# Stansfash/nonstationary-precip

Measured on AMD Instinct MI355X. Metric: dsvi_elbo_steps_per_sec, higher is better.
Workload: dtype f32; 1 GPU; 2-layer DSVI DeepGP (hidden 3->2 + last 2->1), M=1024, S=10, minibatch 4096 (global, split over the GPUs) of synthetic N=1e5 spatio-temporal grid; fwd+ELBO+bwd+Adam; M=1024, S=10, per_gpu_batch=4096, global_batch=4096, N=100000, parallelism=dp1, kzz_cholesky_dtype=f64, hipgraph=True

## Files before the change

nonstationary-precip_amd/csrc/gemm_i8.hip:

```cpp
#include <cstdlib>
#include "common.h"

namespace {

#ifndef NSGP_I8_DMA
#define NSGP_I8_DMA 1
#endif
constexpr int I8_BM = 128, I8_BN = 64, I8_BK = 32;
constexpr int I8_SW = 5;

typedef int v4i __attribute__((ext_vector_type(4)));
typedef int v16i __attribute__((ext_vector_type(16)));

__global__ __launch_bounds__(256) void i8_slice_w_kernel(const double* __restrict__ W, int64_t M, int64_t Mp, int64_t KB,
                                                         signed char* __restrict__ Wd, double* __restrict__ wsc) {
    __shared__ double lds[4];
    const int64_t b = blockIdx.y, m = blockIdx.x;
    signed char* out = Wd + b * (int64_t)I8_SW * KB * 2 * Mp * 16;
    const int64_t plane = KB * 2 * Mp * 16;
    if (m >= M) {
        for (int64_t k = threadIdx.x; k < KB * 32; k += 256)
            for (int a = 0; a < I8_SW; ++a) out[a * plane + ((k >> 5) * 2 + ((k >> 4) & 1)) * Mp * 16 + m * 16 + (k & 15)] = 0;
        return;
    }
    const double* row = W + (b * M + m) * M;
    const auto nmax = [](double a, double c) { return (a > c || a != a) ? a : c; };
    double mx = 0.0;
    for (int64_t k = threadIdx.x; k <= m; k += 256) mx = nmax(fabs(row[k]), mx);
    for (int off = 32; off > 0; off >>= 1) mx = nmax(__shfl_xor(mx, off, 64), mx);
    if ((threadIdx.x & 63) == 0) lds[threadIdx.x >> 6] = mx;
    __syncthreads();
    mx = nmax(nmax(lds[0], lds[1]), nmax(lds[2], lds[3]));
    const bool fin = mx <= 1.7976931348623157e308;
    int e = 0;
    (void)frexp(fin ? mx : 0.0, &e);
    const double rs = (fin && mx > 0.0) ? ldexp(1.0, e) : 1.0;
    if (threadIdx.x == 0) wsc[b * M + m] = fin ? rs / 64.0 : __builtin_nan("");
    const double inv = 64.0 / rs;
    for (int64_t k = threadIdx.x; k < KB * 32; k += 256) {
        double t = (fin && k <= m && k < M) ? row[k] * inv : 0.0;
        const int64_t o = ((k >> 5) * 2 + ((k >> 4) & 1)) * Mp * 16 + m * 16 + (k & 15);
#pragma unroll
        for (int a = 0; a < I8_SW; ++a) {
            const double d = rint(t);
            out[a * plane + o] = (signed char)(int)d;
            t = (t - d) * 128.0;
        }
    }
}

template <int D, int SK>
__global__ __launch_bounds__(256) void i8_rbf_build_kernel(const float* __restrict__ Z, const float* __restrict__ x, int64_t sx,
                                                           const float* __restrict__ ls, const float* __restrict__ os,
                                                           int64_t M, int64_t n, int64_t np, int64_t KB,
                                                           signed char* __restrict__ Kd, double* __restrict__ ksc,
                                                           float* __restrict__ Kf) {
    const int64_t b = blockIdx.z, kb = blockIdx.y;
    const int64_t j = (int64_t)blockIdx.x * 256 + threadIdx.x;
    __shared__ double zs[32][D];
    __shared__ int bad;
    if (threadIdx.x == 0) bad = 0;
    if (threadIdx.x < 32 * D) {
        const int kk = threadIdx.x / D, d = threadIdx.x % D;
        const int64_t k = kb * 32 + kk;
        zs[kk][d] = k < M ? (double)Z[(b * M + k) * D + d] / (double)ls[b * D + d] : 0.0;
    }
    __syncthreads();
    const double osd = (double)os[b];
    bool fin = fabs(osd) <= 1.7976931348623157e308;
#pragma unroll
    for (int d = 0; d < D; ++d) fin = fin && fabs((double)ls[b * D + d]) <= 1.7976931348623157e308;
    int e = 0;
    (void)frexp(fin ? osd : 0.0, &e);
    const double cs = ldexp(1.0, e);
    const double sc = fin ? osd * 64.0 / cs : 0.0;
    if (j < np) {
        double xs[D];
#pragma unroll
        for (int d = 0; d < D; ++d) xs[d] = j < n ? (double)x[b * sx + j * D + d] / (double)ls[b * D + d] : 0.0;
        signed char* out = Kd + b * (int64_t)SK * KB * 2 * np * 16;
        const int64_t plane = KB * 2 * np * 16;
#pragma unroll
        for (int h = 0; h < 2; ++h) {
            int pk[SK][4] = {};
#pragma unroll
            for (int q = 0; q < 16; ++q) {
                const int kk = h * 16 + q;
                double r2 = 0.0;
#pragma unroll
                for (int d = 0; d < D; ++d) { const double df = zs[kk][d] - xs[d]; r2 = __builtin_fma(df, df, r2); }
                const bool in = j < n && kb * 32 + kk < M;
                const bool nan_e = in && r2 != r2;
                if (nan_e) bad = 1;
                const double ev = in ? t_fexp<double>(-0.5 * r2) : 0.0;
                const double evd = nan_e ? 0.0 : ev;
                if (Kf && in) Kf[(b * M + kb * 32 + kk) * n + j] = (float)(osd * ev);
                double t = sc * evd;
#pragma unroll
                for (int s = 0; s < SK; ++s) {
                    const double dg = rint(t);
                    pk[s][q >> 2] |= ((int)dg & 0xFF) << (8 * (q & 3));
                    t = (t - dg) * 128.0;
                }
            }
#pragma unroll
            for (int s = 0; s < SK; ++s) {
                v4i v = {pk[s][0], pk[s][1], pk[s][2], pk[s][3]};
                *reinterpret_cast<v4i*>(out + s * plane + (kb * 2 + h) * np * 16 + j * 16) = v;
            }
        }
    }
    __syncthreads();
    if (threadIdx.x == 0)
        ksc[(b * KB + kb) * gridDim.x + blockIdx.x] = (fin && !bad) ? cs / 64.0 : __builtin_nan("");
}

template <int P64, int SK, int LEV>
__global__ __launch_bounds__(256, 2) void i8_proj_kernel(const signed char* __restrict__ Wd, const double* __restrict__ wsc,
                                                         const signed char* __restrict__ Kd, const double* __restrict__ ksc,
                                                         const float* __restrict__ rv, int64_t M, int64_t n, int64_t Mp,
                                                         int64_t np, int64_t KB, int tiles_n, float* __restrict__ Y,
                                                         void* __restrict__ p0, void* __restrict__ p1, int part_rows) {
    extern __shared__ __attribute__((aligned(16))) unsigned char i8_smem[];
    constexpr int A_STAGE = I8_SW * 2 * I8_BM * 16, B_STAGE = SK * 2 * I8_BN * 16;
    unsigned char* As = i8_smem;
    unsigned char* Bs = i8_smem + 2 * A_STAGE;
    double* Ws = reinterpret_cast<double*>(i8_smem + 2 * (A_STAGE + B_STAGE));
    float* Rs = reinterpret_cast<float*>(Ws + I8_BM);
    const int tid = threadIdx.x, lane = tid & 63, wave = __builtin_amdgcn_readfirstlane(tid >> 6);
    const int wm0 = (wave >> 1) * 64, wn0 = (wave & 1) * 32;
    const int64_t bb = blockIdx.y;
    const int tiles_m = (int)(Mp / I8_BM);
    const int bm = tiles_m - 1 - (int)blockIdx.x / tiles_n;
    const int bn = (int)blockIdx.x % tiles_n;
    const int64_t m0 = (int64_t)bm * I8_BM, n0 = (int64_t)bn * I8_BN;
    int nkb = (int)((m0 + I8_BM) / I8_BK);
    if (nkb > KB) nkb = (int)KB;
    const signed char* Wb = Wd + bb * (int64_t)I8_SW * KB * 2 * Mp * 16;
    const signed char* Kb = Kd + bb * (int64_t)SK * KB * 2 * np * 16;
    const int64_t wplane = KB * 2 * Mp * 16, kplane = KB * 2 * np * 16;

    const signed char* ga[5];
#pragma unroll
    for (int j = 0; j < 5; ++j) {
        const int q = tid + 256 * j;
        const int a = q >> 8, h = (q >> 7) & 1, row = q & 127;
        ga[j] = Wb + a * wplane + (int64_t)h * Mp * 16 + (m0 + row) * 16;
    }
    constexpr int NPB = (SK * 128 + 255) / 256;
    const signed char* gb[NPB];
#pragma unroll
    for (int j = 0; j < NPB; ++j) {
        int q = tid + 256 * j;
        if (q >= SK * 128) q = SK * 128 - 1;
        const int s = q >> 7, h = (q >> 6) & 1, col = q & 63;
        gb[j] = Kb + s * kplane + (int64_t)h * np * 16 + (n0 + col) * 16;
    }
    const int64_t astep = 2 * Mp * 16, bstep = 2 * np * 16;
#if NSGP_I8_DMA
    typedef const __attribute__((address_space(1))) void* gptr_t;
    typedef __attribute__((address_space(3))) void* lptr_t;
    auto dma = [&](int kb, int buf) __attribute__((always_inline)) {
#pragma unroll
        for (int j = 0; j < 5; ++j)
            __builtin_amdgcn_global_load_lds((gptr_t)(ga[j] + (int64_t)kb * astep),
                                             (lptr_t)(As + buf * A_STAGE + (wave * 64 + 256 * j) * 16), 16, 0, 0);
#pragma unroll
        for (int j = 0; j < NPB; ++j)
            if (wave * 64 + 256 * j < SK * 128)
                __builtin_amdgcn_global_load_lds((gptr_t)(gb[j] + (int64_t)kb * bstep),
                                                 (lptr_t)(Bs + buf * B_STAGE + (wave * 64 + 256 * j) * 16), 16, 0, 0);
    };
#endif
    v4i ra[5], rb[NPB];
    auto gload = [&](int kb) __attribute__((always_inline)) {
#pragma unroll
        for (int j = 0; j < 5; ++j) ra[j] = *reinterpret_cast<const v4i*>(ga[j] + (int64_t)kb * astep);
#pragma unroll
        for (int j = 0; j < NPB; ++j) rb[j] = *reinterpret_cast<const v4i*>(gb[j] + (int64_t)kb * bstep);
    };
    auto sstore = [&](int buf) __attribute__((always_inline)) {
#pragma unroll
        for (int j = 0; j < 5; ++j) *reinterpret_cast<v4i*>(As + buf * A_STAGE + (tid + 256 * j) * 16) = ra[j];
#pragma unroll
        for (int j = 0; j < NPB; ++j)
            if (tid + 256 * j < SK * 128) *reinterpret_cast<v4i*>(Bs + buf * B_STAGE + (tid + 256 * j) * 16) = rb[j];
    };

    v16i acc[LEV][2];
#pragma unroll
    for (int l = 0; l < LEV; ++l)
#pragma unroll
        for (int i = 0; i < 2; ++i)
#pragma unroll
            for (int r = 0; r < 16; ++r) acc[l][i][r] = 0;

    const int wave_nkb = __builtin_amdgcn_readfirstlane((int)((m0 + wm0 + 64 + I8_BK - 1) / I8_BK));
    const int half = lane >> 5, lr = lane & 31;
    const int64_t gx = (np + 255) >> 8;
    const double* ks = ksc + bb * KB * gx + (n0 >> 8);
    const float* rvb = rv ? rv + bb * M : nullptr;
#if NSGP_I8_DMA
    dma(0, 0);
#else
    gload(0);
    sstore(0);
#endif
    const double kslot = ks[(int64_t)(tid < nkb ? tid : nkb - 1) * gx];
    const int64_t prow = m0 + (tid & (I8_BM - 1)), crow = prow < M ? prow : M - 1;
    const double wload = wsc[bb * M + crow];
    const float rload = rvb ? rvb[crow] : 0.0f;
    const double wrow = prow < M ? wload : 0.0;
    const float rrow = prow < M ? rload : 0.0f;
    if (tid < I8_BM) { Ws[tid] = wrow; Rs[tid] = rrow; }
#if NSGP_I8_DMA
    asm volatile("s_waitcnt vmcnt(0)" ::: "memory");
#endif
    const double kscale = __syncthreads_or(kslot != kslot) ? __builtin_nan("") : ks[0];
    for (int kb = 0; kb < nkb; ++kb) {
        const int buf = kb & 1;
#if NSGP_I8_DMA
        if (kb + 1 < nkb) dma(kb + 1, buf ^ 1);
#else
        if (kb + 1 < nkb) gload(kb + 1);
#endif
        if (kb < wave_nkb) {
            v4i af[2][2], bf[SK];
#pragma unroll
            for (int s = 0; s < SK; ++s)
                bf[s] = *reinterpret_cast<const v4i*>(Bs + buf * B_STAGE + ((s * 2 + half) * I8_BN + wn0 + lr) * 16);
#pragma unroll
            for (int i = 0; i < 2; ++i)
                af[0][i] = *reinterpret_cast<const v4i*>(As + buf * A_STAGE + ((0 * 2 + half) * I8_BM + wm0 + 32 * i + lr) * 16);
#pragma unroll
            for (int a = 0; a < I8_SW; ++a) {
                if (a + 1 < I8_SW) {
#pragma unroll
                    for (int i = 0; i < 2; ++i)
                        af[(a + 1) & 1][i] = *reinterpret_cast<const v4i*>(
                            As + buf * A_STAGE + (((a + 1) * 2 + half) * I8_BM + wm0 + 32 * i + lr) * 16);
                }
#pragma unroll
                for (int s = 0; s < SK; ++s)
                    if (a + s < LEV) {
#pragma unroll
                        for (int i = 0; i < 2; ++i)
                            acc[a + s][i] = __builtin_amdgcn_mfma_i32_32x32x32_i8(af[a & 1][i], bf[s], acc[a + s][i], 0, 0, 0);
                    }
            }
        }
#if NSGP_I8_DMA
        asm volatile("s_waitcnt vmcnt(0)" ::: "memory");
#else
        if (kb + 1 < nkb) sstore(buf ^ 1);
#endif
        __syncthreads();
    }

    double sdot = 0.0, ssq = 0.0;
    const int64_t col = n0 + wn0 + lr;
#pragma unroll
    for (int i = 0; i < 2; ++i)
#pragma unroll
        for (int r = 0; r < 16; ++r) {
            const int lrow = wm0 + 32 * i + (r & 3) + 8 * (r >> 2) + 4 * half;
            const int64_t row = m0 + lrow;
            const double wr = Ws[lrow];
            const float rr = Rs[lrow];
            double v = (double)acc[LEV - 1][i][r];
#pragma unroll
            for (int l = LEV - 2; l >= 0; --l) v = __builtin_fma(v, 0.0078125, (double)acc[l][i][r]);
            const bool in = row < M && col < n;
            v *= (in ? wr : 0.0) * kscale;
            if (in) Y[(bb * M + row) * n + col] = (float)v;
            sdot += v * ((rvb && in) ? (double)rr : 0.0);
            ssq += v * v;
        }
    sdot += __shfl_xor(sdot, 32, 64);
    ssq += __shfl_xor(ssq, 32, 64);
    double* red = reinterpret_cast<double*>(i8_smem);
    __syncthreads();
    if (lane < 32) {
        red[(0 + (wave >> 1)) * I8_BN + wn0 + lane] = sdot;
        red[(2 + (wave >> 1)) * I8_BN + wn0 + lane] = ssq;
    }
    __syncthreads();
    if (tid < I8_BN && n0 + tid < n) {
        const int64_t o = (bb * part_rows + bm) * n + n0 + tid;
        const double d = red[tid] + red[I8_BN + tid], q = red[2 * I8_BN + tid] + red[3 * I8_BN + tid];
        if (P64) {
            if (p0) reinterpret_cast<double*>(p0)[o] = d;
            reinterpret_cast<double*>(p1)[o] = q;
        } else {
            if (p0) reinterpret_cast<float*>(p0)[o] = (float)d;
            reinterpret_cast<float*>(p1)[o] = (float)q;
        }
    }
}

static inline int64_t i8_mp(int64_t M) { return cdiv64(M, I8_BM) * I8_BM; }
static inline int64_t i8_np(int64_t n) { return cdiv64(n, I8_BN) * I8_BN; }
static inline int64_t i8_kb(int64_t M) { return cdiv64(M, I8_BK); }

}

extern "C" {

int nsgp_i8_supported(int64_t M) { return (M >= 1 && M <= 4096) ? 1 : 0; }
size_t nsgp_i8_w_planes_bytes(int64_t batch, int64_t M) {
    return (batch > 0 && M > 0) ? (size_t)(batch * I8_SW * i8_kb(M) * 2 * i8_mp(M) * 16) : 0;
}
size_t nsgp_i8_k_planes_bytes(int64_t batch, int64_t M, int64_t n, int planes) {
    return (batch > 0 && M > 0 && n > 0 && (planes == 4 || planes == 5)) ? (size_t)(batch * planes * i8_kb(M) * 2 * i8_np(n) * 16) : 0;
}
size_t nsgp_i8_tiles(int64_t M) { return M > 0 ? (size_t)cdiv64(M, I8_BM) : 0; }
size_t nsgp_i8_kscale_count(int64_t batch, int64_t M, int64_t n) {
    return (batch > 0 && M > 0 && n > 0) ? (size_t)(batch * i8_kb(M) * cdiv64(i8_np(n), 256)) : 0;
}

int nsgp_i8_slice_w_f64(const double* W, int64_t batch, int64_t M, void* Wd, double* wscale, void* stream) {
    if (!W) return -1; if (batch < 0) return -2; if (M < 0 || !nsgp_i8_supported(M > 0 ? M : 1)) return -3;
    if (!Wd) return -4; if (!wscale) return -5;
    if (batch == 0 || M == 0) return 0;
    if (batch > 65535) return -2;
    hipLaunchKernelGGL(i8_slice_w_kernel, dim3((unsigned)i8_mp(M), (unsigned)batch), dim3(256), 0, (hipStream_t)stream, W, M,
                       i8_mp(M), i8_kb(M), (signed char*)Wd, wscale);
    return nsgp_launch_status();
}

int nsgp_i8_rbf_build_f32(const float* Z, const float* x, int64_t x_batch_stride, const float* ls, const float* os,
                          int64_t batch, int64_t M, int64_t n, int D, int planes, void* Kd, double* kscale, float* Kzx_f32,
                          void* stream) {
    if (planes != 4 && planes != 5) return -10;
    if (!Z) return -1; if (!x) return -2; if (x_batch_stride < 0) return -3; if (!ls) return -4; if (!os) return -5;
    if (batch < 0) return -6; if (M < 0 || !nsgp_i8_supported(M > 0 ? M : 1)) return -7; if (n < 0) return -8;
    if (D < 1 || D > 4) return -9; if (!Kd) return -10; if (!kscale) return -11;
    if (batch == 0 || M == 0 || n == 0) return 0;
    if (batch > 65535 || i8_kb(M) > 65535) return -6;
    const int64_t np = i8_np(n), KB = i8_kb(M);
    dim3 grid((unsigned)cdiv64(np, 256), (unsigned)KB, (unsigned)batch);
    hipStream_t st = (hipStream_t)stream;
    signed char* kd = (signed char*)Kd;
#define NSGP_I8_BUILD(DD, SS) hipLaunchKernelGGL((i8_rbf_build_kernel<DD, SS>), grid, dim3(256), 0, st, Z, x, x_batch_stride, ls, os, M, n, np, KB, kd, kscale, Kzx_f32)
    if (planes == 4) {
        switch (D) { case 1: NSGP_I8_BUILD(1, 4); break; case 2: NSGP_I8_BUILD(2, 4); break; case 3: NSGP_I8_BUILD(3, 4); break;
                     default: NSGP_I8_BUILD(4, 4); break; }
    } else {
        switch (D) { case 1: NSGP_I8_BUILD(1, 5); break; case 2: NSGP_I8_BUILD(2, 5); break; case 3: NSGP_I8_BUILD(3, 5); break;
                     default: NSGP_I8_BUILD(4, 5); break; }
    }
#undef NSGP_I8_BUILD
    return nsgp_launch_status();
}

int nsgp_svgp_tri_gemm_colstats_i8(const void* Wd, const double* wscale, const void* Kd, const double* kscale,
                                   int planes, const float* rowvec, int64_t batch, int64_t M, int64_t n, float* Y,
                                   void* part_dot, void* part_sq, int64_t part_rows, int partials_f64, void* stream) {
    if (planes != 4 && planes != 5) return -5;
    if (!Wd) return -1; if (!wscale) return -2; if (!Kd) return -3; if (!kscale) return -4;
    if (batch < 0) return -6; if (M < 0 || !nsgp_i8_supported(M > 0 ? M : 1)) return -7; if (n < 0) return -8;
    if (!Y) return -9; if (!part_sq) return -11; if (part_rows < cdiv64(M > 0 ? M : 1, I8_BM)) return -12;
    if (batch == 0 || M == 0 || n == 0) return 0;
    const int64_t Mp = i8_mp(M), np = i8_np(n), KB = i8_kb(M);
    const int64_t tiles_n = np / I8_BN, tiles = (Mp / I8_BM) * tiles_n;
    if (tiles > 2147483647LL || batch > 65535) return -8;
    const size_t lds = 2 * (size_t)(I8_SW * 2 * I8_BM * 16 + planes * 2 * I8_BN * 16) + I8_BM * (sizeof(double) + sizeof(float));
    hipStream_t st = (hipStream_t)stream;
    dim3 grid((unsigned)tiles, (unsigned)batch);
#define NSGP_I8_PROJ(PP, SS) hipLaunchKernelGGL((i8_proj_kernel<PP, SS, (SS == 5 ? 6 : 5)>), grid, dim3(256), lds, st, (const signed char*)Wd, wscale, \
        (const signed char*)Kd, kscale, rowvec, M, n, Mp, np, KB, (int)tiles_n, Y, part_dot, part_sq, (int)part_rows)
    if (planes == 4) { if (partials_f64) NSGP_I8_PROJ(1, 4); else NSGP_I8_PROJ(0, 4); }
    else { if (partials_f64) NSGP_I8_PROJ(1, 5); else NSGP_I8_PROJ(0, 5); }
#undef NSGP_I8_PROJ
    return nsgp_launch_status();
}

}
```

Before: 239.9 steps/s.

## Make int8 projection GEMM persistent with 128x128 tiles and multi-stage DMA pipeline

Reworks the int8 sliced triangular projection kernel into a persistent kernel. It launches one 512-thread workgroup per CU, and each workgroup walks tiles in a serpentine order. The N tile grows from 64 to 128 columns and the inner loop gets a configurable stage pipeline using direct global-to-LDS loads with vmcnt-based waits. The next tile's prologue loads overlap the current tile's epilogue. The aim is to cut launch/tail imbalance and global-load stalls and to raise reuse of the A planes. In exchange it uses more LDS per block, lowers occupancy, and adds hand-written waitcnt and barrier logic.

```diff
diff --git a/nonstationary-precip_amd/csrc/gemm_i8.hip b/nonstationary-precip_amd/csrc/gemm_i8.hip
--- a/nonstationary-precip_amd/csrc/gemm_i8.hip
+++ b/nonstationary-precip_amd/csrc/gemm_i8.hip
@@ -3,10 +3,12 @@
 
 namespace {
 
-#ifndef NSGP_I8_DMA
-#define NSGP_I8_DMA 1
+#ifndef NSGP_I8_STAGES
+#define NSGP_I8_STAGES 2
 #endif
-constexpr int I8_BM = 128, I8_BN = 64, I8_BK = 32;
+constexpr int I8_BM = 128, I8_BN = 128, I8_BK = 32;
+constexpr int I8_NPAD = 64;
+constexpr int I8_STAGES = NSGP_I8_STAGES;
 constexpr int I8_SW = 5;
 
 typedef int v4i __attribute__((ext_vector_type(4)));
@@ -115,192 +117,245 @@
         ksc[(b * KB + kb) * gridDim.x + blockIdx.x] = (fin && !bad) ? cs / 64.0 : __builtin_nan("");
 }
 
+template <int N> __device__ __forceinline__ void i8_vmwait() { asm volatile("s_waitcnt vmcnt(%0)" ::"n"(N) : "memory"); }
+__device__ __forceinline__ void i8_barrier() { asm volatile("s_waitcnt lgkmcnt(0)\n\ts_barrier" ::: "memory"); }
+
 template <int P64, int SK, int LEV>
-__global__ __launch_bounds__(256, 2) void i8_proj_kernel(const signed char* __restrict__ Wd, const double* __restrict__ wsc,
-                                                         const signed char* __restrict__ Kd, const double* __restrict__ ksc,
-                                                         const float* __restrict__ rv, int64_t M, int64_t n, int64_t Mp,
-                                                         int64_t np, int64_t KB, int tiles_n, float* __restrict__ Y,
-                                                         void* __restrict__ p0, void* __restrict__ p1, int part_rows) {
+__global__ __launch_bounds__(512) void i8_proj_kernel(const signed char* __restrict__ Wd, const double* __restrict__ wsc,
+                                                      const signed char* __restrict__ Kd, const double* __restrict__ ksc,
+                                                      const float* __restrict__ rv, int64_t M, int64_t n, int64_t Mp,
+                                                      int64_t np, int64_t KB, int tiles_n, int tiles_row, int total,
+                                                      float* __restrict__ Y, void* __restrict__ p0, void* __restrict__ p1,
+                                                      int part_rows) {
     extern __shared__ __attribute__((aligned(16))) unsigned char i8_smem[];
-    constexpr int A_STAGE = I8_SW * 2 * I8_BM * 16, B_STAGE = SK * 2 * I8_BN * 16;
-    unsigned char* As = i8_smem;
-    unsigned char* Bs = i8_smem + 2 * A_STAGE;
-    double* Ws = reinterpret_cast<double*>(i8_smem + 2 * (A_STAGE + B_STAGE));
+    constexpr int NST = I8_STAGES, DEPTH = NST - 1;
+    constexpr int A_STAGE = I8_SW * 2 * I8_BM * 16, STAGE = A_STAGE + SK * 2 * I8_BN * 16;
+    constexpr int ACH = A_STAGE / 1024, NCH = STAGE / 1024, NJ = (NCH + 7) / 8;
+    static_assert(DEPTH >= 1 && DEPTH <= 3 && 8 * (NJ - 1) < NCH, "chunk schedule");
+    double* red = reinterpret_cast<double*>(i8_smem + NST * STAGE);
+    double* Ws = red + 4 * I8_BN;
     float* Rs = reinterpret_cast<float*>(Ws + I8_BM);
+    int* Fl = reinterpret_cast<int*>(Rs + I8_BM);
     const int tid = threadIdx.x, lane = tid & 63, wave = __builtin_amdgcn_readfirstlane(tid >> 6);
-    const int wm0 = (wave >> 1) * 64, wn0 = (wave & 1) * 32;
-    const int64_t bb = blockIdx.y;
-    const int tiles_m = (int)(Mp / I8_BM);
-    const int bm = tiles_m - 1 - (int)blockIdx.x / tiles_n;
-    const int bn = (int)blockIdx.x % tiles_n;
-    const int64_t m0 = (int64_t)bm * I8_BM, n0 = (int64_t)bn * I8_BN;
-    int nkb = (int)((m0 + I8_BM) / I8_BK);
-    if (nkb > KB) nkb = (int)KB;
-    const signed char* Wb = Wd + bb * (int64_t)I8_SW * KB * 2 * Mp * 16;
-    const signed char* Kb = Kd + bb * (int64_t)SK * KB * 2 * np * 16;
+    const int wm0 = (wave >> 2) * 64, wn0 = (wave & 3) * 32;
+    const int halfl = lane >> 5, lrl = lane & 31;
     const int64_t wplane = KB * 2 * Mp * 16, kplane = KB * 2 * np * 16;
-
-    const signed char* ga[5];
-#pragma unroll
-    for (int j = 0; j < 5; ++j) {
-        const int q = tid + 256 * j;
-        const int a = q >> 8, h = (q >> 7) & 1, row = q & 127;
-        ga[j] = Wb + a * wplane + (int64_t)h * Mp * 16 + (m0 + row) * 16;
-    }
-    constexpr int NPB = (SK * 128 + 255) / 256;
-    const signed char* gb[NPB];
-#pragma unroll
-    for (int j = 0; j < NPB; ++j) {
-        int q = tid + 256 * j;
-        if (q >= SK * 128) q = SK * 128 - 1;
-        const int s = q >> 7, h = (q >> 6) & 1, col = q & 63;
-        gb[j] = Kb + s * kplane + (int64_t)h * np * 16 + (n0 + col) * 16;
-    }
     const int64_t astep = 2 * Mp * 16, bstep = 2 * np * 16;
-#if NSGP_I8_DMA
+    const int64_t gx = (np + 255) >> 8;
+    const bool last_dma = NCH % 8 == 0 || wave + 8 * (NJ - 1) < NCH;
+
+    int bm = 0, nkb = 0, wave_nkb = 0;
+    int64_t bb = 0, m0 = 0, n0 = 0;
+    const signed char* g[NJ];
+    int64_t gstep[NJ];
+    unsigned voffa = 0, voffb = 0;
+    double kslot = 0.0, ks0 = 0.0, wload = 0.0;
+    float rload = 0.0f;
+
     typedef const __attribute__((address_space(1))) void* gptr_t;
     typedef __attribute__((address_space(3))) void* lptr_t;
-    auto dma = [&](int kb, int buf) __attribute__((always_inline)) {
-#pragma unroll
-        for (int j = 0; j < 5; ++j)
-            __builtin_amdgcn_global_load_lds((gptr_t)(ga[j] + (int64_t)kb * astep),
-                                             (lptr_t)(As + buf * A_STAGE + (wave * 64 + 256 * j) * 16), 16, 0, 0);
-#pragma unroll
-        for (int j = 0; j < NPB; ++j)
-            if (wave * 64 + 256 * j < SK * 128)
-                __builtin_amdgcn_global_load_lds((gptr_t)(gb[j] + (int64_t)kb * bstep),
-                                                 (lptr_t)(Bs + buf * B_STAGE + (wave * 64 + 256 * j) * 16), 16, 0, 0);
+    auto dma = [&](int kb, int st) __attribute__((always_inline)) {
+#pragma unroll
+        for (int j = 0; j < NJ; ++j)
+            if (j < NJ - 1 || last_dma) {
+                const signed char* base = g[j] + (int64_t)kb * gstep[j];
+                unsigned voff = wave + 8 * j < ACH ? voffa : voffb;
+                asm volatile("" : "+s"(base), "+v"(voff));
+                __builtin_amdgcn_global_load_lds((gptr_t)(base + voff),
+                                                 (lptr_t)(i8_smem + st * STAGE + (wave + 8 * j) * 1024), 16, 0, 0);
+            }
     };
+    auto wait_stages = [&](int k) __attribute__((always_inline)) {
+        if (k <= 0) i8_vmwait<0>();
+        else if (k == 1) { if (last_dma) i8_vmwait<NJ>(); else i8_vmwait<NJ - 1>(); }
+        else if (k == 2) { if (last_dma) i8_vmwait<2 * NJ>(); else i8_vmwait<2 * (NJ - 1)>(); }
+        else { if (last_dma) i8_vmwait<3 * NJ>(); else i8_vmwait<3 * (NJ - 1)>(); }
+    };
+    auto begin_tile = [&](int t) __attribute__((always_inline)) {
+        const int q = (int)((unsigned)t / (unsigned)tiles_row), r = t - q * tiles_row;
+        bm = (int)(Mp / I8_BM) - 1 - q;
+        bb = (int)((unsigned)r / (unsigned)tiles_n);
+        const int bn = r - (int)bb * tiles_n;
+        m0 = (int64_t)bm * I8_BM, n0 = (int64_t)bn * I8_BN;
+        nkb = (int)((m0 + I8_BM) / I8_BK);
+        if (nkb > KB) nkb = (int)KB;
+        wave_nkb = __builtin_amdgcn_readfirstlane((int)((m0 + wm0 + 64 + I8_BK - 1) / I8_BK));
+        const signed char* Wb = Wd + bb * (int64_t)I8_SW * KB * 2 * Mp * 16;
+        const signed char* Kb = Kd + bb * (int64_t)SK * KB * 2 * np * 16;
+#pragma unroll
+        for (int j = 0; j < NJ; ++j) {
+            int c = wave + 8 * j;
+            if (c >= NCH) c = NCH - 1;
+            if (c < ACH) {
+                g[j] = Wb + (c >> 2) * wplane + (int64_t)((c >> 1) & 1) * Mp * 16 + (m0 + (c & 1) * 64) * 16;
+                gstep[j] = astep;
+            } else {
+                const int cb = c - ACH;
+                g[j] = Kb + (cb >> 2) * kplane + (int64_t)((cb >> 1) & 1) * np * 16;
+                gstep[j] = bstep;
+            }
+        }
+        voffa = (unsigned)lane * 16u;
+        {
+            int64_t col = n0 + (wave & 1) * 64 + lane;
+            if (col >= np) col = np - 1;
+            voffb = (unsigned)col * 16u;
+        }
+#pragma unroll
+        for (int d = 0; d < DEPTH; ++d)
+            if (d < nkb) dma(d, d);
+        const double* ks = ksc + bb * KB * gx + (n0 >> 8);
+        kslot = ks[(int64_t)(tid < nkb ? tid : nkb - 1) * gx];
+        ks0 = ks[0];
+        const int64_t prow = m0 + (tid & (I8_BM - 1)), crow = prow < M ? prow : M - 1;
+        wload = wsc[bb * M + crow];
+        rload = rv ? rv[bb * M + crow] : 0.0f;
+    };
+
+    const int G = (int)gridDim.x, wg = (int)blockIdx.x;
+    const auto tile_of = [&](int j) { return (int64_t)j * G + ((j & 1) ? G - 1 - wg : wg); };
+    int round = 0;
+    begin_tile((int)tile_of(0));
+    for (;;) {
+        {
+            int tid = (int)threadIdx.x;
+            asm volatile("" : "+v"(tid));
+            const int64_t prow = m0 + (tid & (I8_BM - 1));
+            const double wrow = prow < M ? wload : 0.0;
+            const float rrow = prow < M ? rload : 0.0f;
+            if (tid < I8_BM) { Ws[tid] = wrow; Rs[tid] = rrow; }
+            const bool anynan = __builtin_amdgcn_ballot_w64(kslot != kslot) != 0;
+            if (wave < 2 && lane == 0) Fl[wave] = anynan ? 1 : 0;
+        }
+        i8_vmwait<0>();
+        i8_barrier();
+        const double kscale = (Fl[0] | Fl[1]) ? __builtin_nan("") : ks0;
+
+        v16i acc[LEV][2];
+#pragma unroll
+        for (int l = 0; l < LEV; ++l)
+#pragma unroll
+            for (int i = 0; i < 2; ++i)
+#pragma unroll
+                for (int r = 0; r < 16; ++r) acc[l][i][r] = 0;
+
+        int st = 0, stn = DEPTH;
+        for (int kb = 0; kb < nkb; ++kb) {
+            if (kb > 0) {
+                const int ahead = nkb - 1 - kb;
+                wait_stages(ahead < DEPTH - 1 ? ahead : DEPTH - 1);
+                i8_barrier();
+            }
+#if !defined(NSGP_I8_PROBE_NO_STAGING)
+            if (kb + DEPTH < nkb) dma(kb + DEPTH, stn);
 #endif
-    v4i ra[5], rb[NPB];
-    auto gload = [&](int kb) __attribute__((always_inline)) {
-#pragma unroll
-        for (int j = 0; j < 5; ++j) ra[j] = *reinterpret_cast<const v4i*>(ga[j] + (int64_t)kb * astep);
-#pragma unroll
-        for (int j = 0; j < NPB; ++j) rb[j] = *reinterpret_cast<const v4i*>(gb[j] + (int64_t)kb * bstep);
-    };
-    auto sstore = [&](int buf) __attribute__((always_inline)) {
-#pragma unroll
-        for (int j = 0; j < 5; ++j) *reinterpret_cast<v4i*>(As + buf * A_STAGE + (tid + 256 * j) * 16) = ra[j];
-#pragma unroll
-        for (int j = 0; j < NPB; ++j)
-            if (tid + 256 * j < SK * 128) *reinterpret_cast<v4i*>(Bs + buf * B_STAGE + (tid + 256 * j) * 16) = rb[j];
-    };
-
-    v16i acc[LEV][2];
-#pragma unroll
-    for (int l = 0; l < LEV; ++l)
-#pragma unroll
-        for (int i = 0; i < 2; ++i)
-#pragma unroll
-            for (int r = 0; r < 16; ++r) acc[l][i][r] = 0;
-
-    const int wave_nkb = __builtin_amdgcn_readfirstlane((int)((m0 + wm0 + 64 + I8_BK - 1) / I8_BK));
-    const int half = lane >> 5, lr = lane & 31;
-    const int64_t gx = (np + 255) >> 8;
-    const double* ks = ksc + bb * KB * gx + (n0 >> 8);
-    const float* rvb = rv ? rv + bb * M : nullptr;
-#if NSGP_I8_DMA
-    dma(0, 0);
-#else
-    gload(0);
-    sstore(0);
+#if !defined(NSGP_I8_PROBE_NO_MFMA)
+            if (kb < wave_nkb) {
+                const unsigned char* As = i8_smem + st * STAGE;
+                const unsigned char* Bs = As + A_STAGE;
+                const int half = halfl, lr = lrl;
+                v4i af[2][2], bf[SK];
+#pragma unroll
+                for (int s = 0; s < SK; ++s)
+                    bf[s] = *reinterpret_cast<const v4i*>(Bs + ((s * 2 + half) * I8_BN + wn0 + lr) * 16);
+#pragma unroll
+                for (int i = 0; i < 2; ++i)
+                    af[0][i] = *reinterpret_cast<const v4i*>(As + ((0 * 2 + half) * I8_BM + wm0 + 32 * i + lr) * 16);
+#pragma unroll
+                for (int a = 0; a < I8_SW; ++a) {
+                    if (a + 1 < I8_SW) {
+#pragma unroll
+                        for (int i = 0; i < 2; ++i)
+                            af[(a + 1) & 1][i] = *reinterpret_cast<const v4i*>(
+                                As + (((a + 1) * 2 + half) * I8_BM + wm0 + 32 * i + lr) * 16);
+                    }
+#pragma unroll
+                    for (int s = 0; s < SK; ++s)
+                        if (a + s < LEV) {
+#pragma unroll
+                            for (int i = 0; i < 2; ++i)
+                                acc[a + s][i] = __builtin_amdgcn_mfma_i32_32x32x32_i8(af[a & 1][i], bf[s], acc[a + s][i], 0, 0, 0);
+                        }
+                }
+            }
 #endif
-    const double kslot = ks[(int64_t)(tid < nkb ? tid : nkb - 1) * gx];
-    const int64_t prow = m0 + (tid & (I8_BM - 1)), crow = prow < M ? prow : M - 1;
-    const double wload = wsc[bb * M + crow];
-    const float rload = rvb ? rvb[crow] : 0.0f;
-    const double wrow = prow < M ? wload : 0.0;
-    const float rrow = prow < M ? rload : 0.0f;
-    if (tid < I8_BM) { Ws[tid] = wrow; Rs[tid] = rrow; }
-#if NSGP_I8_DMA
-    asm volatile("s_waitcnt vmcnt(0)" ::: "memory");
-#endif
-    const double kscale = __syncthreads_or(kslot != kslot) ? __builtin_nan("") : ks[0];
-    for (int kb = 0; kb < nkb; ++kb) {
-        const int buf = kb & 1;
-#if NSGP_I8_DMA
-        if (kb + 1 < nkb) dma(kb + 1, buf ^ 1);
-#else
-        if (kb + 1 < nkb) gload(kb + 1);
-#endif
-        if (kb < wave_nkb) {
-            v4i af[2][2], bf[SK];
-#pragma unroll
-            for (int s = 0; s < SK; ++s)
-                bf[s] = *reinterpret_cast<const v4i*>(Bs + buf * B_STAGE + ((s * 2 + half) * I8_BN + wn0 + lr) * 16);
+            st = st + 1 == NST ? 0 : st + 1;
+            stn = stn + 1 == NST ? 0 : stn + 1;
+        }
+
+        const int64_t m0e = m0, n0e = n0, bbe = bb;
+        const int bme = bm;
+        ++round;
+        const int64_t tn = tile_of(round);
+        const bool more = tn < total;
+        if (more) {
+            i8_barrier();
+            begin_tile((int)tn);
+        }
+
+        {
+            const int64_t m0 = m0e, n0 = n0e, bb = bbe;
+            const int bm = bme;
+            const float* rvb = rv ? rv + bb * M : nullptr;
+            double sdot = 0.0, ssq = 0.0;
+            int half = halfl, lr = lrl;
+            asm volatile("" : "+v"(half), "+v"(lr));
+            const int64_t col = n0 + wn0 + lr;
 #pragma unroll
             for (int i = 0; i < 2; ++i)
-                af[0][i] = *reinterpret_cast<const v4i*>(As + buf * A_STAGE + ((0 * 2 + half) * I8_BM + wm0 + 32 * i + lr) * 16);
-#pragma unroll
-            for (int a = 0; a < I8_SW; ++a) {
-                if (a + 1 < I8_SW) {
-#pragma unroll
-                    for (int i = 0; i < 2; ++i)
-                        af[(a + 1) & 1][i] = *reinterpret_cast<const v4i*>(
-                            As + buf * A_STAGE + (((a + 1) * 2 + half) * I8_BM + wm0 + 32 * i + lr) * 16);
+#pragma unroll
+                for (int r = 0; r < 16; ++r) {
+                    const int lrow = wm0 + 32 * i + (r & 3) + 8 * (r >> 2) + 4 * half;
+                    const int64_t row = m0 + lrow;
+                    const double wr = Ws[lrow];
+                    const float rr = Rs[lrow];
+                    double v = (double)acc[LEV - 1][i][r];
+#pragma unroll
+                    for (int l = LEV - 2; l >= 0; --l) v = __builtin_fma(v, 0.0078125, (double)acc[l][i][r]);
+                    const bool in = row < M && col < n;
+                    v *= (in ? wr : 0.0) * kscale;
+                    if (in) Y[(bb * M + row) * n + col] = (float)v;
+                    sdot += v * ((rvb && in) ? (double)rr : 0.0);
+                    ssq += v * v;
                 }
-#pragma unroll
-                for (int s = 0; s < SK; ++s)
-                    if (a + s < LEV) {
-#pragma unroll
-                        for (int i = 0; i < 2; ++i)
-                            acc[a + s][i] = __builtin_amdgcn_mfma_i32_32x32x32_i8(af[a & 1][i], bf[s], acc[a + s][i], 0, 0, 0);
-                    }
-            }
-        }
-#if NSGP_I8_DMA
-        asm volatile("s_waitcnt vmcnt(0)" ::: "memory");
-#else
-        if (kb + 1 < nkb) sstore(buf ^ 1);
-#endif
-        __syncthreads();
-    }
-
-    double sdot = 0.0, ssq = 0.0;
-    const int64_t col = n0 + wn0 + lr;
-#pragma unroll
-    for (int i = 0; i < 2; ++i)
-#pragma unroll
-        for (int r = 0; r < 16; ++r) {
-            const int lrow = wm0 + 32 * i + (r & 3) + 8 * (r >> 2) + 4 * half;
-            const int64_t row = m0 + lrow;
-            const double wr = Ws[lrow];
-            const float rr = Rs[lrow];
-            double v = (double)acc[LEV - 1][i][r];
-#pragma unroll
-            for (int l = LEV - 2; l >= 0; --l) v = __builtin_fma(v, 0.0078125, (double)acc[l][i][r]);
-            const bool in = row < M && col < n;
-            v *= (in ? wr : 0.0) * kscale;
-            if (in) Y[(bb * M + row) * n + col] = (float)v;
-            sdot += v * ((rvb && in) ? (double)rr : 0.0);
-            ssq += v * v;
-        }
-    sdot += __shfl_xor(sdot, 32, 64);
-    ssq += __shfl_xor(ssq, 32, 64);
-    double* red = reinterpret_cast<double*>(i8_smem);
-    __syncthreads();
-    if (lane < 32) {
-        red[(0 + (wave >> 1)) * I8_BN + wn0 + lane] = sdot;
-        red[(2 + (wave >> 1)) * I8_BN + wn0 + lane] = ssq;
-    }
-    __syncthreads();
-    if (tid < I8_BN && n0 + tid < n) {
-        const int64_t o = (bb * part_rows + bm) * n + n0 + tid;
-        const double d = red[tid] + red[I8_BN + tid], q = red[2 * I8_BN + tid] + red[3 * I8_BN + tid];
-        if (P64) {
-            if (p0) reinterpret_cast<double*>(p0)[o] = d;
-            reinterpret_cast<double*>(p1)[o] = q;
-        } else {
-            if (p0) reinterpret_cast<float*>(p0)[o] = (float)d;
-            reinterpret_cast<float*>(p1)[o] = (float)q;
-        }
+            sdot += __shfl_xor(sdot, 32, 64);
+            ssq += __shfl_xor(ssq, 32, 64);
+            if (half == 0) {
+                red[(0 + (wave >> 2)) * I8_BN + wn0 + lr] = sdot;
+                red[(2 + (wave >> 2)) * I8_BN + wn0 + lr] = ssq;
+            }
+            i8_barrier();
+            const int tid = wave * 64 + 32 * half + lr;
+            if (tid < I8_BN && n0 + tid < n) {
+                const int64_t o = (bb * part_rows + bm) * n + n0 + tid;
+                const double d = red[tid] + red[I8_BN + tid], q = red[2 * I8_BN + tid] + red[3 * I8_BN + tid];
+                if (P64) {
+                    if (p0) reinterpret_cast<double*>(p0)[o] = d;
+                    reinterpret_cast<double*>(p1)[o] = q;
+                } else {
+                    if (p0) reinterpret_cast<float*>(p0)[o] = (float)d;
+                    reinterpret_cast<float*>(p1)[o] = (float)q;
+                }
+            }
+        }
+        if (!more) break;
     }
 }
 
 static inline int64_t i8_mp(int64_t M) { return cdiv64(M, I8_BM) * I8_BM; }
-static inline int64_t i8_np(int64_t n) { return cdiv64(n, I8_BN) * I8_BN; }
+static inline int64_t i8_np(int64_t n) { return cdiv64(n, I8_NPAD) * I8_NPAD; }
 static inline int64_t i8_kb(int64_t M) { return cdiv64(M, I8_BK); }
+
+static int i8_cu_count() {
+    static std::mutex mu;
+    static int cus[64] = {};
+    int dev = 0;
+    (void)hipGetDevice(&dev);
+    std::lock_guard<std::mutex> lk(mu);
+    int& c = cus[dev & 63];
+    if (c <= 0 && (hipDeviceGetAttribute(&c, hipDeviceAttributeMultiprocessorCount, dev) != hipSuccess || c <= 0)) c = 256;
+    return c;
+}
 
 }
 
@@ -362,13 +417,22 @@
     if (!Y) return -9; if (!part_sq) return -11; if (part_rows < cdiv64(M > 0 ? M : 1, I8_BM)) return -12;
     if (batch == 0 || M == 0 || n == 0) return 0;
     const int64_t Mp = i8_mp(M), np = i8_np(n), KB = i8_kb(M);
-    const int64_t tiles_n = np / I8_BN, tiles = (Mp / I8_BM) * tiles_n;
-    if (tiles > 2147483647LL || batch > 65535) return -8;
-    const size_t lds = 2 * (size_t)(I8_SW * 2 * I8_BM * 16 + planes * 2 * I8_BN * 16) + I8_BM * (sizeof(double) + sizeof(float));
+    const int64_t tiles_n = cdiv64(n, I8_BN), tiles_row = batch * tiles_n, total = (Mp / I8_BM) * tiles_row;
+    if (total > 2147483647LL || batch > 65535) return -8;
+    int64_t G = i8_cu_count();
+#ifdef NSGP_I8_PROBE_ONE_TILE
+    G = total;
+#endif
+    if (G > total) G = total;
+    const size_t lds = (size_t)I8_STAGES * (I8_SW * 2 * I8_BM * 16 + planes * 2 * I8_BN * 16) + 4 * I8_BN * sizeof(double) +
+                       I8_BM * (sizeof(double) + sizeof(float)) + 16;
     hipStream_t st = (hipStream_t)stream;
-    dim3 grid((unsigned)tiles, (unsigned)batch);
-#define NSGP_I8_PROJ(PP, SS) hipLaunchKernelGGL((i8_proj_kernel<PP, SS, (SS == 5 ? 6 : 5)>), grid, dim3(256), lds, st, (const signed char*)Wd, wscale, \
-        (const signed char*)Kd, kscale, rowvec, M, n, Mp, np, KB, (int)tiles_n, Y, part_dot, part_sq, (int)part_rows)
+#define NSGP_I8_PROJ(PP, SS) do { \
+        auto kern = i8_proj_kernel<PP, SS, (SS == 5 ? 6 : 5)>; \
+        nsgp_opt_in_lds((const void*)kern, lds); \
+        hipLaunchKernelGGL(kern, dim3((unsigned)G), dim3(512), lds, st, (const signed char*)Wd, wscale, (const signed char*)Kd, \
+                           kscale, rowvec, M, n, Mp, np, KB, (int)tiles_n, (int)tiles_row, (int)total, Y, part_dot, part_sq, (int)part_rows); \
+    } while (0)
     if (planes == 4) { if (partials_f64) NSGP_I8_PROJ(1, 4); else NSGP_I8_PROJ(0, 4); }
     else { if (partials_f64) NSGP_I8_PROJ(1, 5); else NSGP_I8_PROJ(0, 5); }
 #undef NSGP_I8_PROJ
```

Result: no change. 240.8 steps/s, median of 6 (+0.4%).
